# airframesio/aero-cli

Measured on AMD Instinct MI355X. Metric: Msamples/s demod+Viterbi, 10500bps OQPSK, 1/2/4/8 GPU; ACARS frames bit-exact vs ref, higher is better.
Workload: dtype f64

## Files before the change

### aero-cli_amd/build.py

```python
import argparse
import concurrent.futures as cf
import os
import shutil
import subprocess
import sys

HERE = os.path.dirname(os.path.abspath(__file__))
ROOT = os.path.dirname(HERE)
CSRC = os.path.join(HERE, 'csrc')
BUILD = os.path.join(HERE, 'build')
ENGINE_SO = os.path.join(HERE, 'libaero_engine.so')
SYNTH_SO = os.path.join(ROOT, 'tools', 'libaero_synth.so')
ORACLE_DIR = os.path.join(ROOT, 'oracle')

ARCH = os.environ.get('AERO_OFFLOAD_ARCH', 'gfx950')
HIPCC = os.environ.get('HIPCC', shutil.which('hipcc') or '/opt/rocm/bin/hipcc')
FP = ['-ffp-contract=off', '-fno-fast-math']
HIP_FLAGS = ['-O3', '-std=c++17', '-fPIC', '--offload-arch=' + ARCH] + FP
CXX_FLAGS = ['-O2', '-std=c++17', '-fPIC', '-Wall'] + FP

HIP_SRCS = ['demod_oqpsk.hip', 'demod_msk.hip', 'coarse.hip', 'aerol.hip', 'engine.hip', 'chan.hip', 'burst.hip', 'burst_msk.hip',
            'burst_engine.hip', 'cchan.hip', 'slot_reset.hip', 'slot_copy.hip']
CXX_SRCS = ['tables_host.cpp', 'acars_host.cpp', 'chan_blob.cpp']
FILE_FLAGS = {'burst.hip': ['-mllvm', '-disable-machine-licm'],
# ... 41 lines not shown
        for f in [ex.submit(_run, t) for t in tasks]:
            f.result()
    if tasks or _stale(out, objs):
        _run([HIPCC, '--offload-arch=' + ARCH, '-shared', '-fPIC', '-o', out] + objs)
    return out


def build_synth():
    src = os.path.join(ROOT, 'tools', 'aero_synth.cpp')
    if _stale(SYNTH_SO, [src]):
        _run(['g++', '-O2', '-std=c++17', '-fPIC', '-shared', '-o', SYNTH_SO, src, '-lm'])
    return SYNTH_SO


MATHHOST_SO = os.path.join(ROOT, 'tools', 'libaero_mathhost.so')
FFTSIM_SO = os.path.join(ROOT, 'tools', 'libfft_chain_sim.so')


def build_fftsim():
    src = os.path.join(ROOT, 'tools', 'fft_chain_sim.cpp')
    if _stale(FFTSIM_SO, [src, os.path.join(CSRC, 'fft_layout.h')]):
        _run(['g++', '-O2', '-std=c++17', '-fPIC', '-shared', '-ffp-contract=off', '-o', FFTSIM_SO, src])
    return FFTSIM_SO


SCHEDSIM_SO = os.path.join(ROOT, 'tools', 'libcoarse_sched_sim.so')


def build_schedsim():
    src = os.path.join(ROOT, 'tools', 'coarse_sched_sim.cpp')
    if _stale(SCHEDSIM_SO, [src, os.path.join(CSRC, 'coarse_sched.h')]):
        _run(['g++', '-O2', '-std=c++17', '-Wall', '-fPIC', '-shared', '-o', SCHEDSIM_SO, src])
    return SCHEDSIM_SO


CHANSLOTS_SO = os.path.join(ROOT, 'tools', 'libchan_slots_sim.so')


def build_chanslots():
    src = os.path.join(ROOT, 'tools', 'chan_slots_sim.cpp')
    if _stale(CHANSLOTS_SO, [src, os.path.join(CSRC, 'chan_slots.h')]):
        _run(['g++', '-O2', '-std=c++17', '-Wall', '-fPIC', '-shared', '-o', CHANSLOTS_SO, src])
    return CHANSLOTS_SO


def build_mathhost():
    src = os.path.join(ROOT, 'tools', 'mathhost.cpp')
    deps = [src, os.path.join(CSRC, 'aero_math.h'), os.path.join(CSRC, 'aero_glibc_tables.h')]
    if _stale(MATHHOST_SO, deps):
        _run(['g++', '-O2', '-std=c++17', '-fPIC', '-shared', '-ffp-contract=off', '-o', MATHHOST_SO, src, '-lm'])
    return MATHHOST_SO


HOSTCHECK_SO = os.path.join(ROOT, 'tools', 'libaero_hostcheck.so')
HOSTCHECK_SRCS = [os.path.join(ROOT, 'tools', 'hostcheck.cpp'), os.path.join(CSRC, 'acars_host.cpp'),
                  os.path.join(CSRC, 'chan_blob.cpp'), os.path.join(CSRC, 'tables_host.cpp')]


def build_hostcheck(out=HOSTCHECK_SO, extra=()):
    deps = HOSTCHECK_SRCS + [os.path.join(CSRC, h) for h in ('acars_host.h', 'chan_blob.h', 'tables_host.h')]
    if _stale(out, deps):
        _run(['g++'] + CXX_FLAGS + list(extra) + ['-shared', '-o', out] + HOSTCHECK_SRCS + ['-lm'])
    return out


def build_oracle():
# ... 59 lines not shown
    base = ['g++', '-O1', '-std=c++17', '-fPIC'] + FP + SAN
    out = {}
    jobsl = []
    def lib(name, srcs, extra=()):
        so = os.path.join(d, name)
        out[name] = so
        if _stale(so, srcs + [os.path.join(CSRC, 'aero_math.h'), os.path.join(CSRC, 'aero_glibc_tables.h')]):
            jobsl.append(base + list(extra) + ['-shared', '-o', so] + srcs + ['-lm'])
    lib('liboracle.so', [os.path.join(ORACLE_DIR, 'aero_oracle.cpp'), os.path.join(ORACLE_DIR, 'pub_oracle.cpp')])
    lib('libaero_synth.so', [os.path.join(ROOT, 'tools', 'aero_synth.cpp')])
    lib('libaero_mathhost.so', [os.path.join(ROOT, 'tools', 'mathhost.cpp')])
    lib('libaero_hostcheck.so', HOSTCHECK_SRCS)
    hs = [os.path.join(HOST, s) for s in HOST_COMMON]
    lib(os.path.join('bin', 'libaero_host.so'), [os.path.join(HOST, 'host_capi.cpp')] + hs[:2])
    for name, srcs in HOST_BINS.items():
        exe = os.path.join(bindir, name)
        out[name] = exe
        allsrc = [os.path.join(HOST, s) for s in srcs] + hs
        if _stale(exe, allsrc + [ENGINE_SO]):
            jobsl.append(base + ['-o', exe] + allsrc + [ENGINE_SO, '-Wl,-rpath,' + HERE, '-rdynamic', '-ldl',
                                                          '-lpthread'])
    with cf.ThreadPoolExecutor(max_workers=max(1, jobs)) as ex:
        for f in [ex.submit(_run, t) for t in jobsl]:
            f.result()
    return out


def build_all(jobs=4):
    build_oracle()
    build_synth()
    build_mathhost()
    build_fftsim()
    build_schedsim()
    build_chanslots()
    build_hostcheck()
    so = build_engine(jobs)
    build_diag(jobs)
    build_host(jobs)
    return so


DIAG_VARIANTS = {'handoff_fail': ['AERO_X_HANDOFF_FAIL']}


def build_diag(jobs=4):
    return [build_engine(jobs, variant=v, defines=d) for v, d in DIAG_VARIANTS.items()]


DROP_VARIANTS = {'drop%d' % k: ['AERO_X_DROP=%d' % k] for k in (1, 2, 4, 8)}


def build_drop(jobs=4):
    return [build_engine(jobs, variant=v, defines=d) for v, d in DROP_VARIANTS.items()]


BLIBM_VARIANTS = {'blibm%d' % k: ['AERO_X_BURST_LIBM=%d' % k] for k in (1, 2, 3)}


def build_blibm(jobs=4):
    return [build_engine(jobs, variant=v, defines=d) for v, d in BLIBM_VARIANTS.items()]


COARSE_VARIANTS = {'cisline': ['AERO_X_CISLINE'], 'noyread': ['AERO_X_NOYREAD']}


def build_coarse(jobs=4):
# ... 34 lines not shown
```

### aero-cli_amd/csrc/aero_math.h

```cpp
#pragma once
#include <stdint.h>

#if defined(__HIPCC__)
#include <hip/hip_runtime.h>
#define AERO_HD __host__ __device__ __forceinline__
#define AERO_TABLE_DECL static __host__ __device__ constexpr
#else
#include <math.h>
#define AERO_HD static inline
#define AERO_TABLE_DECL static constexpr
#endif

#include "aero_glibc_tables.h"

namespace aero {

AERO_HD uint64_t d2u(double x) { return __builtin_bit_cast(uint64_t, x); }
AERO_HD double u2d(uint64_t u) { return __builtin_bit_cast(double, u); }
AERO_HD uint32_t hiw(double x) { return (uint32_t)(d2u(x) >> 32); }
AERO_HD uint32_t low(double x) { return (uint32_t)d2u(x); }
AERO_HD double sethi(double x, uint32_t hi) {
  return u2d((d2u(x) & 0xffffffffULL) | ((uint64_t)hi << 32));
}
AERO_HD double mkd(uint32_t hi, uint32_t lo) { return u2d(((uint64_t)hi << 32) | lo); }
// ... 643 lines not shown
  const double du = div_r((a - vb) - vvb, b, r);
  const bool pos = x > 0;
  const bool prim = pos && gt;
  const bool cpi = !pos && !(ay > ax);
  const double K = cpi ? AERO_G_OPI : AERO_G_HPI, K1 = cpi ? AERO_G_OPI1 : AERO_G_HPI1;
  const double s = (!pos && ay > ax) ? 1.0 : -1.0;
  const double vs = u * u;
  const double poly = g_atan2_poly(vs);
  const double uv = u * vs;
  const double zp_s = u + fma(uv, poly, du);
  const double zz = uv * poly;
  const double ts = K + s * u;
  const double cor = (K - ts) + s * u;
  const double zg_s = (((cor + K1) + s * du) + s * zz) + ts;
  int row = g_atan2_row(u);
  row = row < 0 ? 0 : row;
  const double *c = cij[row];
  const double t3 = u - c[0];
  const double v = t3 + du;
  const double dv = (__builtin_fabs(t3) > __builtin_fabs(du)) ? ((t3 - v) + du) : ((du - v) + t3);
  double p3 = fma(v, c[6], c[5]);
  p3 = fma(v, p3, c[4]);
  p3 = fma(v, p3, c[3]);
  const double zp_t = fma(v, c[2], fma(dv, c[2], (v * v) * p3)) + c[1];
  const double P = fma(v, p3, c[2]);
  const double zg_t = (K + s * c[1]) + fma(s * v, P, K1);
  const double z = u < AERO_G_INV16 ? (prim ? zp_s : zg_s) : (prim ? zp_t : zg_t);
  return __builtin_copysign(z, y);
#else
  return aero_atan2_t(y, x, cij);
#endif
}

AERO_HD double aero_log(double x) {
  const uint64_t ix = d2u(x);
  const uint32_t top = (uint32_t)(ix >> 48);
  if (ix - 0x3fee000000000000ULL < 0x3090000000000ULL) {
    if (ix == 0x3ff0000000000000ULL) return 0.0;
    const double *B = aero_g_log_poly1;
    const double r = x - 1.0;
    const double r2 = r * r, r3 = r * r2;
    double p9 = fma(r3, B[10], fma(r2, B[9], fma(r, B[8], B[7])));
    p9 = fma(p9, r3, fma(r2, B[6], fma(r, B[5], B[4])));
    const double p = fma(p9, r3, fma(r2, B[3], fma(r, B[2], B[1])));
    const double rhi = fma(-AERO_G_TWO27, r, fma(r, AERO_G_TWO27, r));
    const double rlo = r - rhi;
    const double hi = fma(rhi * rhi, B[0], r);
    double lo = fma(rhi * rhi, B[0], r - hi);
    lo = fma(B[0] * rlo, r + rhi, lo);
    return hi + fma(p, r3, lo);
  }
  uint64_t jx = ix;
  if (top - 0x0010u >= 0x7ff0u - 0x0010u) {
    if ((ix << 1) == 0) return -1.0 / 0.0;
    if (ix == 0x7ff0000000000000ULL) return x;
    if ((top & 0x8000u) || (top & 0x7ff0u) == 0x7ff0u) return (x - x) / (x - x);
    jx = d2u(x * 0x1p52) - (52ULL << 52);
  }
  const uint64_t tmp = jx - 0x3fe6000000000000ULL;
  const int i = (int)((tmp >> 45) & 127);
  const int k = (int)((int64_t)tmp >> 52);
  const double z = u2d(jx - (tmp & (0xfffULL << 52)));
  const double invc = aero_g_log_tab[i][0], logc = aero_g_log_tab[i][1];
  const double r = fma(z, invc, -1.0);
  const double kd = (double)k;
  const double w = fma(kd, AERO_G_LN2HI, logc);
  const double hi = w + r;
  const double lo = fma(kd, AERO_G_LN2LO, (w - hi) + r);
  const double r2 = r * r;
  const double *A = aero_g_log_poly;
  const double q = fma(fma(r, A[4], A[3]), r2, fma(r, A[2], A[1]));
  return fma(r * r2, q, fma(r2, A[0], lo)) + hi;
}

AERO_HD double aero_log10(double x) {
  const double two54 = 0x1p54;
  int64_t ix = (int64_t)d2u(x);
  int64_t k;
  if (ix > 0x000fffffffffffffLL) {
    k = -1023;
  } else {
    if ((ix & 0x7fffffffffffffffLL) == 0) return -two54 / __builtin_fabs(x);
    if (ix < 0) return (x - x) / (x - x);
    x *= two54;
    ix = (int64_t)d2u(x);
    k = -1023 - 54;
  }
  if ((uint64_t)ix > 0x7fefffffffffffffULL) return x + x;
  k += ix >> 52;
  const int64_t i = (int64_t)((uint64_t)k >> 63);
  const double y = (double)(k + i);
  x = u2d((uint64_t)(ix & 0x000fffffffffffffLL) | ((uint64_t)(0x3ff - i) << 52));
  const double z = y * AERO_G_LOG10_2LO + aero_log(x) * AERO_G_IVLN10;
  return z + y * AERO_G_LOG10_2HI;
}

}
```

### aero-cli_amd/csrc/coarse.hip

```cpp
#include <hip/hip_runtime.h>

#include <type_traits>

#include "aero_math.h"
#include "coarse_sched.h"
#include "engine_common.h"
#include "fft_chain.h"

namespace aero {

#ifdef AERO_X_OCML
#define CO_HYPOT ::hypot
#define CO_HYPOT_NR ::hypot
#define CO_LOG10 ::log10
#else
#define CO_HYPOT aero_hypot
#define CO_HYPOT_NR aero_hypot_nr
#define CO_LOG10 aero_log10
#endif

template <int M>
struct CoarseK;
template <>
struct CoarseK<MODE_OQPSK> {
  static constexpr int LOG2N = 14, HOPN = 4096, START = 3584, STOP = 12800, ILO = 4608, IHI = 11776, EPB = 1792;
  static constexpr int YLO = 2815, YHI = 13568;
  static constexpr double FS = 48000.0;
};
template <>
struct CoarseK<MODE_C8400> {
  static constexpr int LOG2N = 14, HOPN = 4096, START = 3584, STOP = 12800, ILO = 4608, IHI = 11776, EPB = 1434;
  static constexpr int YLO = 2815, YHI = 13568;
  static constexpr double FS = 48000.0;
};
template <int FS>
struct MskCoarseBins;
template <>
struct MskCoarseBins<12000> {
  static constexpr int START = 614, STOP = 7578, ILO = 3482, IHI = 4710, EPB = 205;
};
template <>
struct MskCoarseBins<24000> {
  static constexpr int START = 307, STOP = 7885, ILO = 3789, IHI = 4403, EPB = 102;
};
template <>
struct MskCoarseBins<48000> {
  static constexpr int START = 154, STOP = 8038, ILO = 3942, IHI = 4250, EPB = 51;
};
template <int M>
struct CoarseK {
  using B = MskCoarseBins<msk_fs(M)>;
  static constexpr int LOG2N = 13, HOPN = 2048, START = B::START, STOP = B::STOP, ILO = B::ILO, IHI = B::IHI,
                       EPB = B::EPB;
  static constexpr int YLO = MSK_YLO, YHI = MSK_YHI;
  static_assert(ILO - EPB - 1 >= YLO && IHI - 1 + EPB + 1 <= YHI, "fold search inside the kept y bins");
  static constexpr double FS = (double)msk_fs(M);
};

struct CoarseBins {
  int start, stop, ilo, ihi, epb;
  double fs;
};
template <int M>
__device__ __forceinline__ CoarseBins coarse_bins(const DevState &S) {
  using K = CoarseK<M>;
// ... 147 lines not shown
__device__ __forceinline__ HopPro load_pro(const DevState &S, int C, int c) {
  HopPro p;
  p.filled = S.ls[LS_FILLED * C + c];
  p.zero_before = S.ls[LS_ZERO_BEFORE * C + c];
  p.hops_done = S.is[IS_HOPS_DONE * C + c];
  p.yreset = S.is[IS_YRESET * C + c];
  return p;
}
__device__ __forceinline__ HopPro uni(const HopPro &p) {
  return {uni(p.filled), uni(p.zero_before), uni(p.hops_done), uni(p.yreset)};
}

struct HopEpi {
  double mse, m2f, m2s, mcf, mcs;
  int ecd, countdown2, countdown, iter, scans, steps, hop_n;
};
__device__ __forceinline__ HopEpi load_epi(const DevState &S, int C, int c) {
  HopEpi e;
  e.mse = S.ds[DS_MSE * C + c];
  e.m2f = S.ds[DS_M2_FREQ * C + c];
  e.m2s = S.ds[DS_M2_STEP * C + c];
  e.mcf = S.ds[DS_MC_FREQ * C + c];
  e.mcs = S.ds[DS_MC_STEP * C + c];
  e.ecd = S.is[IS_EMPTYCD * C + c];
  e.countdown2 = S.is[IS_COUNTDOWN2 * C + c];
  e.countdown = S.is[IS_COUNTDOWN * C + c];
  e.iter = S.is[IS_HUNT_ITER * C + c];
  e.scans = S.is[IS_HUNT_SCANS * C + c];
  e.steps = S.is[IS_HUNT_STEPS * C + c];
  e.hop_n = S.hop_n[c];
  return e;
}

template <int M>
__global__ __launch_bounds__(1 << (CoarseK<M>::LOG2N - 4), CoarseK<M>::LOG2N == 13 ? 4 : 1) void coarse_kernel(DevState S, DevTables T, int nch) {
  using K = CoarseK<M>;
  const CoarseBins KB = coarse_bins<M>(S);
  constexpr int L = K::LOG2N, N = 1 << L, FT = N / 16, PADDED = N + N / 16;
  constexpr int YLEN = K::YHI - K::YLO + 1;
  constexpr bool PERSIST = L == 14;
  __shared__ double lds[PADDED];
  __shared__ double2 s_tw[TwLds<L>::LEN];
  __shared__ double red_v[FT / 64];
  __shared__ int red_i[FT / 64];
  const int wave = uni((int)threadIdx.x >> 6);
  const int C = S.C;
  const int wgs = (int)gridDim.x, wg = (int)blockIdx.x;
  const int iters = csched::iters(nch, wgs, wg);
#ifdef AERO_X_STAMPS
  unsigned long long cst_[CSTAMP_N] = {}, ctime_ = __builtin_amdgcn_s_memtime();
  const unsigned long long cstart_ = ctime_;
#endif
  bool have_tw = false;
#pragma unroll 1
  for (int k0 = 0; k0 < iters; k0 += csched::BATCH) {
    bool due = false;
    if (csched::lane_has(iters, k0, lane_now())) {
      const int cc = csched::channel(wgs, wg, k0 + lane_now());
      const long long nsamp = S.ls[LS_NSAMP * C + cc];
      const long long avail = S.ls[LS_AVAIL * C + cc];
      const long long nkk = (long long)K::HOPN * (S.is[IS_HOPS_DONE * C + cc] + 1) - 1;
      due = nsamp == nkk && avail > nkk;
    }
    unsigned long long mask = __ballot(due);
    HopPro pro{};
    bool have_pro = false;
#pragma unroll 1
    while (mask) {
      auto tnow = [&]() { return wave * 64 + lane_now(); };
      int t = PERSIST ? tnow() : (int)threadIdx.x;
      const int c = csched::channel(wgs, wg, k0 + csched::first(mask));
      mask = csched::rest(mask);
      if (!have_pro) pro = uni(load_pro(S, C, c));
      const long long filled = pro.filled, zero_before = pro.zero_before;
      const int hops_done = pro.hops_done, yreset = pro.yreset;
      const long long nk = (long long)K::HOPN * (hops_done + 1) - 1;
      int fixj = -1;
      uint32_t fixw = 0;
      if (filled <= nk) {
        const double mc_ptr = S.ds[DS_MC_PTR * C + c];
        int tint = (int)mc_ptr;
        if (tint >= WTSIZE) tint = 0;
        if (tint < 0) tint = WTSIZE - 1;
        const int16_t xs = S.pcm[(nk & (S.pcm_cap - 1)) * C + c];
        fixw = (uint32_t)tint | ((uint32_t)(uint16_t)xs << 16);
        fixj = (int)(nk & (N - 1));
        if (t == 0) {
          S.cring[(size_t)c * N + fixj] = fixw;
          S.ls[LS_FILLED * C + c] = nk + 1;
        }
      }
      CSTAMP(0);

      if (!have_tw) {
        load_tw_lds<L>(s_tw, T.tw, t, FT);
        have_tw = true;
      }
      uint32_t *ring_lds = reinterpret_cast<uint32_t *>(lds);
      const uint32_t *ring = S.cring + (size_t)c * N;
      if constexpr (PERSIST) {
#pragma unroll
        for (int i = 0; i < N / FT; ++i) {
          const int j = t + i * FT;
          const uint32_t w = ring[j];
          ring_lds[j + (j >> 4)] = j == fixj ? fixw : w;
        }
      } else {
        for (int j = t; j < N; j += FT) {
          const uint32_t w = ring[j];
          ring_lds[j + (j >> 4)] = j == fixj ? fixw : w;
        }
      }
      __syncthreads();
      CSTAMP(1);
      double2 x[16];
      const long long s0 = nk - (N - 1);
      double2 cs[16];
      double dval[16];
#pragma unroll
      for (int i = 0; i < 16; ++i) {
        const int q = (int)((s0 + bitrev<L>(epos<L, 0>(t, i))) & (N - 1));
        const uint32_t w = ring_lds[q + (q >> 4)];
        dval[i] = ((double)(int16_t)(w >> 16)) / 32768.0;
#ifdef AERO_X_CISLINE
        cs[i] = T.cis[w & 0x7];
#else
        cs[i] = T.cis[w & 0xFFFF];
#endif
      }
#pragma unroll
      for (int i = 0; i < 16; ++i) asm volatile("" : "+v"(cs[i].x), "+v"(cs[i].y));
#pragma unroll
      for (int i = 0; i < 16; ++i) {
        const long long s = s0 + bitrev<L>(epos<L, 0>(t, i));
        x[i] = s < zero_before ? make_double2(0.0, 0.0) : make_double2(cs[i].x * dval[i], cs[i].y * dval[i]);
      }
      __syncthreads();
      CSTAMP(2);
      if constexpr (PERSIST) t = tnow();
      chain::fft<L, true, false>(x, t, lds, T.tw, s_tw, T.twg);
      CSTAMP(3);
      if constexpr (PERSIST) t = tnow();
      const int bin_t = chain::out_bin_thread<L>(t);
#pragma unroll
      for (int i = 0; i < 16; ++i) {
        const int p = bin_t | chain::out_bin_reg<L>(i);
        if constexpr (M == MODE_C8400) {
          const double w = T.cwin[i * FT + t];
          x[i] = make_double2(x[i].x * w, x[i].y * w);
        } else {
          if (p >= KB.start && p <= KB.stop) x[i] = make_double2(0.0, 0.0);
        }
      }
      if constexpr (PERSIST) t = tnow();
      chain::fft<L, false, true>(x, t, lds, T.twi, s_tw, T.twgi);
#pragma unroll
      for (int i = 0; i < 16; ++i) {
        const double r = x[i].x * x[i].x - x[i].y * x[i].y;
        const double im = 2.0 * (x[i].x * x[i].y);
        x[i] = make_double2(r, im);
      }
      CSTAMP(4);
      if constexpr (PERSIST) t = tnow();
      chain::fft<L, false, false>(x, t, lds, T.tw, s_tw, T.twg);
      CSTAMP(5);
      if constexpr (PERSIST) t = tnow();
      double *yg = S.y + (size_t)c * YLEN;
#ifdef AERO_X_NOYREAD
      auto yload = [&](int k) { return 20.0 + 0.0 * k; };
#else
      auto yload = [&](int k) { return (k < YLEN && !yreset) ? yg[k] : 20.0; };
#endif
      double yp0 = yload(t), yp1 = yload(t + FT);
      double *ylds = lds;
      auto ypad = [](int q) { return fftl::ypadn<6>(q); };
      bool nr = true;
#pragma unroll
      for (int i = 0; i < 16; ++i) {
        const double a = fabs(x[i].x), b = fabs(x[i].y);
        nr = nr && a <= 0x1p200 && b <= 0x1p200 && (a >= 0x1p-200 || b >= 0x1p-200);
      }
      if (__all(nr)) {
#pragma unroll
        for (int i = 0; i < 16; ++i) {
          const int yi = (bin_t | chain::out_bin_reg<L>(i)) ^ (N / 2);
          if (yi >= K::YLO && yi <= K::YHI) ylds[ypad(yi - K::YLO)] = CO_HYPOT_NR(x[i].x, x[i].y);
        }
      } else {
#pragma unroll
        for (int i = 0; i < 16; ++i) {
          const int yi = (bin_t | chain::out_bin_reg<L>(i)) ^ (N / 2);
          if (yi >= K::YLO && yi <= K::YHI) ylds[ypad(yi - K::YLO)] = CO_HYPOT(x[i].x, x[i].y);
        }
      }
      double yp2 = yload(t + 2 * FT);
      __syncthreads();
      CSTAMP(6);
      have_pro = mask != 0;
      HopPro pn{};
      if (have_pro) pn = load_pro(S, C, csched::channel(wgs, wg, k0 + csched::first(mask)));
      HopEpi ep{};
      if (PERSIST && t < 64) ep = load_epi(S, C, c);
#pragma unroll 1
      for (int k = t; k < YLEN; k += FT) {
        const double yold = yp0;
        yp0 = yp1;
        yp1 = yp2;
        yp2 = yload(k + 3 * FT);
        const double ynew = yold * 0.9 + 0.1 * 10 * CO_LOG10(fmax(ylds[ypad(k)], 1.0));
        yg[k] = ynew;
        ylds[ypad(k)] = ynew;
      }
      __syncthreads();
      CSTAMP(7);
      double bv = 0.0;
      int bi = 0x7fffffff;
      for (int r = 0;; ++r) {
        const int i = KB.ilo + t + FT * r;
        if (i >= KB.ihi) break;
        double val = 0;
        for (int j = -1; j <= 1; j++)
          val += (ylds[ypad(i - KB.epb - j - K::YLO)] + ylds[ypad(i + KB.epb + j - K::YLO)]);
        if (val > bv) {
          bv = val;
          bi = i;
        }
      }
      for (int off = 32; off > 0; off >>= 1) {
        const double ov = __shfl_down(bv, off, 64);
        const int oi = __shfl_down(bi, off, 64);
        if (ov > bv || (ov == bv && oi < bi)) {
          bv = ov;
          bi = oi;
        }
      }
      if ((t & 63) == 0) {
        red_v[t >> 6] = bv;
        red_i[t >> 6] = bi;
      }
      if (have_pro) pro = uni(pn);
      __syncthreads();
      CSTAMP(8);
      if (t == 0) {
        if constexpr (!PERSIST) ep = load_epi(S, C, c);
        for (int w = 1; w < FT / 64; ++w) {
          if (red_v[w] > bv || (red_v[w] == bv && red_i[w] < bi)) {
            bv = red_v[w];
            bi = red_i[w];
          }
        }
        const int zmaxloc = (bv > 0.0) ? bi : N / 2;
        const double nfft = (double)N;
        const double freq_offset_est = -((double)(zmaxloc - nfft / 2)) * (KB.fs / nfft) * 0.5;
        double est;
        int ecd = ep.ecd;
        if (ecd <= 0) {
          est = freq_offset_est;
        } else {
          ecd--;
          est = 0;
        }

        double *ds = S.ds;
        int *is = S.is;
        const double mse = ep.mse;
        HopCtl h;
        h.m2f = ep.m2f;
        h.m2s = ep.m2s;
        h.mcf = ep.mcf;
        h.mcs = ep.mcs;
        h.countdown2 = ep.countdown2;
        h.countdown = ep.countdown;
        h.ecd = ecd;
        h.yres_next = 0;
        h.zb = zero_before;
// ... 27 lines not shown
          hr[2] = h.m2f;
          hr[3] = h.mcf;
          hr[4] = mse;
          hr[5] = gotasignal ? 1.0 : 0.0;
        }
        S.hop_n[c] = hn + 1;
      }
      CSTAMP(9);
#ifdef AERO_X_STAMPS
      cst_[CSTAMP_N - 1]++;
#endif
      if constexpr (!PERSIST) break;
    }
    if constexpr (!PERSIST) break;
  }
#ifdef AERO_X_STAMPS
  if (wave * 64 + lane_now() == 0 && cst_[CSTAMP_N - 1]) {
    cst_[10] = __builtin_amdgcn_s_memtime() - cstart_;
    for (int k = 0; k < CSTAMP_N; ++k) atomicAdd(&g_cstamps[k], cst_[k]);
  }
#endif
}

void coarse_read_stamps(unsigned long long *out) {
#ifdef AERO_X_STAMPS
  (void)hipMemcpyFromSymbol(out, HIP_SYMBOL(g_cstamps), sizeof(unsigned long long) * CSTAMP_N);
  unsigned long long z[CSTAMP_N] = {0};
  (void)hipMemcpyToSymbol(HIP_SYMBOL(g_cstamps), z, sizeof z);
#else
  for (int k = 0; k < CSTAMP_N; ++k) out[k] = 0;
#endif
}

void launch_coarse(hipStream_t st, int mode, const DevState &S, const DevTables &T, int nch, int grid) {
  const dim3 pg(csched::grid(nch, grid < 1 ? 1 : grid));
  switch (mode) {
    case MODE_OQPSK: hipLaunchKernelGGL(coarse_kernel<MODE_OQPSK>, pg, dim3(1024), 0, st, S, T, nch); break;
    case MODE_C8400: hipLaunchKernelGGL(coarse_kernel<MODE_C8400>, pg, dim3(1024), 0, st, S, T, nch); break;
    case MODE_MSK600: hipLaunchKernelGGL(coarse_kernel<MODE_MSK600>, dim3(nch), dim3(512), 0, st, S, T, nch); break;
    case MODE_MSK1200: hipLaunchKernelGGL(coarse_kernel<MODE_MSK1200>, dim3(nch), dim3(512), 0, st, S, T, nch); break;
    case MODE_MSK600_24K:
      hipLaunchKernelGGL(coarse_kernel<MODE_MSK600_24K>, dim3(nch), dim3(512), 0, st, S, T, nch);
      break;
    case MODE_MSK600_48K:
      hipLaunchKernelGGL(coarse_kernel<MODE_MSK600_48K>, dim3(nch), dim3(512), 0, st, S, T, nch);
      break;
    case MODE_MSK1200_12K:
      hipLaunchKernelGGL(coarse_kernel<MODE_MSK1200_12K>, dim3(nch), dim3(512), 0, st, S, T, nch);
      break;
    case MODE_MSK1200_48K:
      hipLaunchKernelGGL(coarse_kernel<MODE_MSK1200_48K>, dim3(nch), dim3(512), 0, st, S, T, nch);
      break;
    default:
      hipLaunchKernelGGL(coarse_kernel<MODE_MSKG600>, dim3(nch), dim3(512), 0, st, S, T, nch);
      break;
  }
}

}
```

### aero-cli_amd/csrc/engine.hip

```cpp
#include <hip/hip_runtime.h>

#include <algorithm>
#include <cmath>
#include <complex>
#include <cstdio>
#include <cstdlib>
#include <cstring>
#include <atomic>
#include <chrono>
#include <climits>
#include <deque>
#include <condition_variable>
#include <functional>
#include <mutex>
#include <new>
#include <map>
#include <memory>
#include <string>
#include <set>
#include <thread>
#include <type_traits>
#include <vector>

#include "../../include/aero_engine.h"
#include "acars_host.h"
#include "burst_engine.h"
#include "aero_math.h"
#include "chan_blob.h"
#include "engine_common.h"
#include "fft_layout.h"
#include "host_pool.h"
#include "engine_internal.h"
#include "slot_copy.h"
#include "slot_reset.h"
#include "tables_host.h"

namespace aero {
void launch_demod(hipStream_t, const DevState &, const DevTables &, int, int, bool, bool);
void upload_demod_constants(const double *, const DelayDesc *, const double *, const double *, const double *,
                            const double *);
void launch_demod_msk(hipStream_t, int, const DevState &, const DevTables &, int, int, bool);
void upload_msk_constants(const double *);
void demod_read_stamps(unsigned long long *);
void coarse_read_stamps(unsigned long long *);
void viterbi_read_stamps(unsigned long long *);
void burst_read_stamps(unsigned long long *);
void launch_coarse(hipStream_t, int, const DevState &, const DevTables &, int, int);
void launch_frame(hipStream_t, int, const DevState &, int);
void launch_viterbi(hipStream_t, int, const DevState &, const DevTables &, int, int);
void launch_prefilter_c(hipStream_t, const DevState &, const DevTables &, const void *, int);
void launch_demod_c(hipStream_t, const DevState &, const DevTables &, int, bool);
void upload_c_constants(const DelayDesc *);
int c_prejob_bytes();
void launch_reset_slots(hipStream_t, void *, const ResetSeg *, int, const int *, const int *, int, const ResetInit *,
                        unsigned long long);
}

using namespace aero;

namespace {

constexpr int GENERIC_GROUP_CAP = 256;
constexpr long long PCM_CAP = 65536;
constexpr int PT_CAP = 4096;
constexpr int HOP_CAP = 64;

#define HIPCHK(x)                                   \
  do {                                              \
    hipError_t err__ = (x);                         \
    if (err__ != hipSuccess) {                      \
      fprintf(stderr, "aero_engine: %s failed: %s\n", #x, hipGetErrorString(err__)); \
      return AERO_E_HIP;                            \
    }                                               \
  } while (0)

__global__ void pcm_scatter_kernel(int16_t *ring, int C, long long capm, const int16_t *src, long long n, long long ld,
                                   int nch, int c0, long long start) {
  const long long total = n * nch;
  for (long long k = blockIdx.x * (long long)blockDim.x + threadIdx.x; k < total;
       k += (long long)gridDim.x * blockDim.x) {
// ... 49 lines not shown

struct TimingSlot {
  double ms = 0;
  long launches = 0;
};

struct HostTimer {
  std::map<std::string, TimingSlot> *t;
  const char *name;
  std::chrono::steady_clock::time_point t0;
  HostTimer(std::map<std::string, TimingSlot> *tm, const char *n) : t(tm), name(n) {
    if (t) t0 = std::chrono::steady_clock::now();
  }
  ~HostTimer() {
    if (!t) return;
    auto &slot = (*t)[name];
    slot.ms += std::chrono::duration<double, std::milli>(std::chrono::steady_clock::now() - t0).count();
    slot.launches++;
  }
};
#define HT_CAT2(a, b) a##b
#define HT_CAT(a, b) HT_CAT2(a, b)
#define HOST_TIMER(e, n) HostTimer HT_CAT(_ht_, __LINE__)(((e)->flags & AERO_F_TIMING) ? &(e)->timing : nullptr, n)

}


struct Group {
  ~Group();
  int mode = MODE_OQPSK;
  int gid = 0;
  int wide_max = 0;
  int coarse_grid = 1;
  ModeGeom g{};
  int device = 0, flags = 0, C = 0, nch = 0;
  std::string tag;
  hipStream_t st = nullptr;
  DevState S{};
  DevTables T{};
  void *pool = nullptr;
  size_t pool_bytes = 0;
  HostPool *hpool = nullptr;
  std::vector<aero_channel_cfg> cfg;
  std::vector<int> gch;
  std::vector<int> free_slots;
  std::vector<int> reset_pending;
  std::vector<uint8_t> reset_wait;
  std::vector<ResetSeg> reset_plan;
  ResetSeg *d_reset_plan = nullptr;
  ResetInit *d_reset_init = nullptr;
  int *d_reset_slots = nullptr, *pin_reset_slots = nullptr;
  hipEvent_t reset_ev = nullptr;
  bool reset_done = false, reset_ready = false;
  uint64_t reset_launches = 0;
  SlotCopier copier;
  std::vector<ResetSeg> slot_plan;
  std::vector<long long> avail, nsamp, hops;
  std::vector<std::unique_ptr<PChannelHost>> host;
  std::vector<std::vector<uint8_t>> infofield;
  std::vector<std::vector<int16_t>> soft_hold;
  std::vector<std::vector<double>> hop_hold, pt_hold;
  std::vector<std::vector<uint8_t>> blk_hold, frame_hold;
  std::vector<long long> soft_seen;
  std::vector<long long> hop_base;
  int job_out = JOB_OUT;
  std::vector<std::deque<long long>> msg_end;
// ... 678 lines not shown
          waited = true;
        }
        jt[ncj++] = {c, 0, e->pre_end[c], e->msg_end[c].front()};
        e->pre_end[c] = e->msg_end[c].front();
        e->msg_end[c].pop_front();
      }
      if (ncj) e->next_cjob = (kcj + 1) % Group::NPIN;
    }
    for (int c = 0; c < e->nch; c++) {
      const long long boundary = HOPN * (e->hops[c] + 1) - 1;
      if (e->nsamp[c] == boundary && e->avail[c] > boundary) {
        e->hops[c]++;
        any_hop = true;
      }
    }
    for (int c = 0; c < e->nch; c++) {
      const long long boundary = HOPN * (e->hops[c] + 1) - 1;
      long long end = std::min(e->avail[c], boundary);
      if (!flush && e->avail[c] <= boundary) end = e->nsamp[c];
      if (cch) end = std::min(e->pre_end[c], boundary);
      if (end > e->nsamp[c]) {
        e->processed += (uint64_t)(end - e->nsamp[c]);
        e->nsamp[c] = end;
        progress = true;
      }
    }
    if (!any_hop && !progress && !ncj) {
      *more = false;
      return AERO_OK;
    }
    hipEvent_t a, b;
    if (any_hop) {
      ev_begin(e, "coarse", a, b);
      launch_coarse(e->st, e->mode, e->S, e->T, e->nch, e->coarse_grid);
      ev_end(e, b);
    }
    if (int rc = issue_viterbi(e)) return rc;
    if (ncj) {
      HIPCHK(hipMemcpyAsync(e->d_cjobs[kcj], e->pin_cjobs[kcj], (size_t)c_prejob_bytes() * ncj,
                            hipMemcpyHostToDevice, e->st));
      HIPCHK(hipEventRecord(e->cjob_ev[kcj], e->st));
      ev_begin(e, "prefilter", a, b);
      launch_prefilter_c(e->st, e->S, e->T, e->d_cjobs[kcj], ncj);
      ev_end(e, b);
      HIPCHK(hipGetLastError());
    }
    if (!progress) return AERO_OK;
    ev_begin(e, "demod", a, b);
    if (cch)
      launch_demod_c(e->st, e->S, e->T, e->nch, (e->flags & AERO_F_TRACE_PT) != 0);
    else if (e->mode == MODE_OQPSK)
      launch_demod(e->st, e->S, e->T, e->nch, flush, (e->flags & AERO_F_TRACE_PT) != 0, e->nch <= e->wide_max);
    else
      launch_demod_msk(e->st, e->mode, e->S, e->T, e->nch, flush, e->nch <= e->wide_max);
    ev_end(e, b);
    if (int rc = note_consumed(e)) return rc;
    if (int rc = frame_round(e, flush, trace)) return rc;
    if (flush && e->S.dcd_tick)
      if (int rc = frame_round(e, flush, trace)) return rc;
  }
  return AERO_OK;
}

int frame_round(Group *e, int flush, bool trace) {
  hipEvent_t a, b;
  {
    const int si = e->next_slot;
// ... 121 lines not shown
  const double nfft = MSK_NFFT, hzperbin = (double)fs / nfft, lockingbw = 900.0, fb = 600.0;
  const double startbin = std::max(std::round(lockingbw / hzperbin), 1.0);
  m.start = (int)startbin;
  m.stop = (int)(nfft - startbin);
  m.epb = (int)std::round(fb / (2.0 * hzperbin));
  m.ilo = (int)std::round((-lockingbw / hzperbin) + ((double)(MSK_NFFT / 2)));
  m.ihi = (int)std::round((lockingbw / hzperbin) + ((double)(MSK_NFFT / 2)));
  return m.ilo - m.epb - 1 >= MSK_YLO && m.ihi - 1 + m.epb + 1 <= MSK_YHI && m.ilo < m.ihi;
}

constexpr int WIDE_MAX_DEFAULT = 4096;

int group_create(aero_engine *E, int mode, int gid, int fs, std::unique_ptr<Group> &out) {
  std::unique_ptr<Group> e(new Group());
  e->mode = mode;
  e->gid = gid;
  e->device = E->device;
  e->flags = E->flags;
  e->hpool = E->hpool.get();
  MskGen mg{};
  if (mode != MODE_OQPSK && mode != MODE_C8400) {
    if (!msk_gen_consts(msk_generic(mode) ? fs : msk_fs(mode), mg)) return AERO_E_RATE;
  }
  {
    const char *w = getenv(mode == MODE_OQPSK ? "AERO_OQPSK_WIDE" : "AERO_MSK_WIDE");
    e->wide_max = w ? atoi(w) : WIDE_MAX_DEFAULT;
    const char *cg = getenv("AERO_COARSE_GRID");
    int cus = 0;
    if (cg)
      cus = atoi(cg);
    else
      HIPCHK(hipDeviceGetAttribute(&cus, hipDeviceAttributeMultiprocessorCount, e->device));
    e->coarse_grid = std::max(cus, 1);
  }
  if (msk_generic(mode)) {
    e->g = msk_geom(msk_bitrate(mode), fs);
    e->tag = "msk" + std::to_string(msk_bitrate(mode)) + "_" + std::to_string(fs) + "_";
  } else if (mode == MODE_C8400) {
    e->g = mode_geom(mode);
    e->tag = "c8400_";
    e->job_out = JOB_OUT_C;
  } else {
    static const char *const tags[MODE_COUNT] = {"", "msk600_", "msk1200_", "msk600_24k_", "msk600_48k_",
                                                  "msk1200_12k_", "msk1200_48k_"};
    e->g = mode_geom(mode);
    e->tag = tags[mode];
  }
  e->C = (E->capacity(msk_generic(mode) ? mode : gid, msk_generic(mode) ? fs : 0) + 63) & ~63;
  if (msk_generic(mode)) e->C = std::min(e->C, GENERIC_GROUP_CAP);
  DevState S{};
  DevTables T{};
  const size_t bytes = layout(S, T, mode, e->g, e->C, e->flags, nullptr) + 4096;
  if (hipMalloc(&e->pool, bytes) != hipSuccess) return AERO_E_NOMEM;
  e->pool_bytes = bytes;
  HIPCHK(hipMemset(e->pool, 0, bytes));
  layout(e->S, e->T, mode, e->g, e->C, e->flags, reinterpret_cast<char *>(e->pool));
  e->S.mg = mg;
  HIPCHK(hipStreamCreateWithFlags(&e->st, hipStreamNonBlocking));
  if (hipHostMalloc(&e->h_err, 64, hipHostMallocMapped | hipHostMallocCoherent) != hipSuccess) return AERO_E_NOMEM;
  *e->h_err = 0;
  HIPCHK(hipHostGetDevicePointer((void **)&e->h_err_dev, e->h_err, 0));
  e->S.err = e->h_err_dev;
  for (auto &sl : e->slot) {
    if (hipMalloc(&sl.d_n, 64) != hipSuccess) return AERO_E_NOMEM;
    if (hipHostMalloc(&sl.h_out, (size_t)e->job_out * e->C, hipHostMallocMapped | hipHostMallocCoherent) != hipSuccess)
      return AERO_E_NOMEM;
// ... 1566 lines not shown
```

Measured before the change: 9013.

## Overlap next channel's ring load and gather with coarse spectrum tail

```diff
diff --git a/aero-cli_amd/build.py b/aero-cli_amd/build.py
--- a/aero-cli_amd/build.py
+++ b/aero-cli_amd/build.py
@@ -97,6 +97,16 @@
     if _stale(SCHEDSIM_SO, [src, os.path.join(CSRC, 'coarse_sched.h')]):
         _run(['g++', '-O2', '-std=c++17', '-Wall', '-fPIC', '-shared', '-o', SCHEDSIM_SO, src])
     return SCHEDSIM_SO
+
+
+LDSSIM_SO = os.path.join(ROOT, 'tools', 'libcoarse_lds_sim.so')
+
+
+def build_ldssim():
+    src = os.path.join(ROOT, 'tools', 'coarse_lds_sim.cpp')
+    if _stale(LDSSIM_SO, [src, os.path.join(CSRC, 'coarse_lds.h')]):
+        _run(['g++', '-O2', '-std=c++17', '-Wall', '-fPIC', '-shared', '-o', LDSSIM_SO, src])
+    return LDSSIM_SO
 
 
 CHANSLOTS_SO = os.path.join(ROOT, 'tools', 'libchan_slots_sim.so')
@@ -222,6 +232,7 @@
     build_mathhost()
     build_fftsim()
     build_schedsim()
+    build_ldssim()
     build_chanslots()
     build_hostcheck()
     so = build_engine(jobs)
diff --git a/aero-cli_amd/csrc/aero_math.h b/aero-cli_amd/csrc/aero_math.h
--- a/aero-cli_amd/csrc/aero_math.h
+++ b/aero-cli_amd/csrc/aero_math.h
@@ -699,7 +699,7 @@
 #endif
 }
 
-AERO_HD double aero_log(double x) {
+AERO_HD double aero_log_tab(double x, const double *tab) {
   const uint64_t ix = d2u(x);
   const uint32_t top = (uint32_t)(ix >> 48);
   if (ix - 0x3fee000000000000ULL < 0x3090000000000ULL) {
@@ -728,7 +728,7 @@
   const int i = (int)((tmp >> 45) & 127);
   const int k = (int)((int64_t)tmp >> 52);
   const double z = u2d(jx - (tmp & (0xfffULL << 52)));
-  const double invc = aero_g_log_tab[i][0], logc = aero_g_log_tab[i][1];
+  const double invc = tab[2 * i], logc = tab[2 * i + 1];
   const double r = fma(z, invc, -1.0);
   const double kd = (double)k;
   const double w = fma(kd, AERO_G_LN2HI, logc);
@@ -740,7 +740,9 @@
   return fma(r * r2, q, fma(r2, A[0], lo)) + hi;
 }
 
-AERO_HD double aero_log10(double x) {
+AERO_HD double aero_log(double x) { return aero_log_tab(x, &aero_g_log_tab[0][0]); }
+
+AERO_HD double aero_log10_tab(double x, const double *tab) {
   const double two54 = 0x1p54;
   int64_t ix = (int64_t)d2u(x);
   int64_t k;
@@ -758,8 +760,9 @@
   const int64_t i = (int64_t)((uint64_t)k >> 63);
   const double y = (double)(k + i);
   x = u2d((uint64_t)(ix & 0x000fffffffffffffLL) | ((uint64_t)(0x3ff - i) << 52));
-  const double z = y * AERO_G_LOG10_2LO + aero_log(x) * AERO_G_IVLN10;
+  const double z = y * AERO_G_LOG10_2LO + aero_log_tab(x, tab) * AERO_G_IVLN10;
   return z + y * AERO_G_LOG10_2HI;
 }
-
-}
+AERO_HD double aero_log10(double x) { return aero_log10_tab(x, &aero_g_log_tab[0][0]); }
+
+}
diff --git a/aero-cli_amd/csrc/coarse.hip b/aero-cli_amd/csrc/coarse.hip
--- a/aero-cli_amd/csrc/coarse.hip
+++ b/aero-cli_amd/csrc/coarse.hip
@@ -3,6 +3,7 @@
 #include <type_traits>
 
 #include "aero_math.h"
+#include "coarse_lds.h"
 #include "coarse_sched.h"
 #include "engine_common.h"
 #include "fft_chain.h"
@@ -13,10 +14,12 @@
 #define CO_HYPOT ::hypot
 #define CO_HYPOT_NR ::hypot
 #define CO_LOG10 ::log10
+#define CO_LOG10_TAB(x, tab) ::log10(x)
 #else
 #define CO_HYPOT aero_hypot
 #define CO_HYPOT_NR aero_hypot_nr
 #define CO_LOG10 aero_log10
+#define CO_LOG10_TAB(x, tab) aero_log10_tab(x, tab)
 #endif
 
 template <int M>
@@ -24,13 +27,13 @@
 template <>
 struct CoarseK<MODE_OQPSK> {
   static constexpr int LOG2N = 14, HOPN = 4096, START = 3584, STOP = 12800, ILO = 4608, IHI = 11776, EPB = 1792;
-  static constexpr int YLO = 2815, YHI = 13568;
+  static constexpr int YLO = clds::YLO14, YHI = clds::YHI14;
   static constexpr double FS = 48000.0;
 };
 template <>
 struct CoarseK<MODE_C8400> {
   static constexpr int LOG2N = 14, HOPN = 4096, START = 3584, STOP = 12800, ILO = 4608, IHI = 11776, EPB = 1434;
-  static constexpr int YLO = 2815, YHI = 13568;
+  static constexpr int YLO = clds::YLO14, YHI = clds::YHI14;
   static constexpr double FS = 48000.0;
 };
 template <int FS>
@@ -244,17 +247,47 @@
   return e;
 }
 
-template <int M>
+template <int L, int YLEN, bool OVL>
+struct CoarseLds {
+  double *lds;
+  double2 *s_tw;
+  double *red_v;
+  int *red_i;
+  uint32_t *img;
+  double *logtab;
+};
+template <int L, int YLEN, bool OVL>
+__device__ __forceinline__ CoarseLds<L, YLEN, OVL> coarse_lds() {
+  using LM = clds::Map<L, YLEN, OVL>;
+  static_assert(LM::TWLEN == TwLds<L>::LEN && clds::ypad(12345) == fftl::ypadn<6>(12345), "coarse_lds.h restates these");
+  if constexpr (OVL) {
+    __shared__ __attribute__((aligned(16))) unsigned char raw[LM::TOTAL];
+    return {reinterpret_cast<double *>(raw + LM::LDS_OFF), reinterpret_cast<double2 *>(raw + LM::TW_OFF),
+            reinterpret_cast<double *>(raw + LM::REDV_OFF), reinterpret_cast<int *>(raw + LM::REDI_OFF),
+            reinterpret_cast<uint32_t *>(raw + LM::IMG_OFF), reinterpret_cast<double *>(raw + LM::LOGTAB_OFF)};
+  } else {
+    __shared__ double lds[LM::PADDED];
+    __shared__ double2 s_tw[LM::TWLEN];
+    __shared__ double red_v[LM::FT / 64];
+    __shared__ int red_i[LM::FT / 64];
+    static_assert(sizeof lds + sizeof s_tw + sizeof red_v + sizeof red_i == LM::TOTAL, "coarse_lds.h describes this");
+    return {lds, s_tw, red_v, red_i, nullptr, nullptr};
+  }
+}
+
+template <int M, bool OVL = false>
 __global__ __launch_bounds__(1 << (CoarseK<M>::LOG2N - 4), CoarseK<M>::LOG2N == 13 ? 4 : 1) void coarse_kernel(DevState S, DevTables T, int nch) {
   using K = CoarseK<M>;
   const CoarseBins KB = coarse_bins<M>(S);
-  constexpr int L = K::LOG2N, N = 1 << L, FT = N / 16, PADDED = N + N / 16;
+  constexpr int L = K::LOG2N, N = 1 << L, FT = N / 16;
   constexpr int YLEN = K::YHI - K::YLO + 1;
   constexpr bool PERSIST = L == 14;
-  __shared__ double lds[PADDED];
-  __shared__ double2 s_tw[TwLds<L>::LEN];
-  __shared__ double red_v[FT / 64];
-  __shared__ int red_i[FT / 64];
+  static_assert(PERSIST || !OVL, "the overlapped head belongs to the persistent walk");
+  const auto sm = coarse_lds<L, YLEN, OVL>();
+  double *const lds = sm.lds;
+  double2 *const s_tw = sm.s_tw;
+  double *const red_v = sm.red_v;
+  int *const red_i = sm.red_i;
   const int wave = uni((int)threadIdx.x >> 6);
   const int C = S.C;
   const int wgs = (int)gridDim.x, wg = (int)blockIdx.x;
@@ -277,6 +310,8 @@
     unsigned long long mask = __ballot(due);
     HopPro pro{};
     bool have_pro = false;
+    bool pre = false;
+    double2 x[16];
 #pragma unroll 1
     while (mask) {
       auto tnow = [&]() { return wave * 64 + lane_now(); };
@@ -287,68 +322,78 @@
       const long long filled = pro.filled, zero_before = pro.zero_before;
       const int hops_done = pro.hops_done, yreset = pro.yreset;
       const long long nk = (long long)K::HOPN * (hops_done + 1) - 1;
-      int fixj = -1;
-      uint32_t fixw = 0;
-      if (filled <= nk) {
-        const double mc_ptr = S.ds[DS_MC_PTR * C + c];
-        int tint = (int)mc_ptr;
-        if (tint >= WTSIZE) tint = 0;
-        if (tint < 0) tint = WTSIZE - 1;
-        const int16_t xs = S.pcm[(nk & (S.pcm_cap - 1)) * C + c];
-        fixw = (uint32_t)tint | ((uint32_t)(uint16_t)xs << 16);
-        fixj = (int)(nk & (N - 1));
-        if (t == 0) {
-          S.cring[(size_t)c * N + fixj] = fixw;
-          S.ls[LS_FILLED * C + c] = nk + 1;
-        }
-      }
-      CSTAMP(0);
-
-      if (!have_tw) {
-        load_tw_lds<L>(s_tw, T.tw, t, FT);
-        have_tw = true;
-      }
-      uint32_t *ring_lds = reinterpret_cast<uint32_t *>(lds);
-      const uint32_t *ring = S.cring + (size_t)c * N;
-      if constexpr (PERSIST) {
-#pragma unroll
-        for (int i = 0; i < N / FT; ++i) {
-          const int j = t + i * FT;
-          const uint32_t w = ring[j];
-          ring_lds[j + (j >> 4)] = j == fixj ? fixw : w;
-        }
-      } else {
-        for (int j = t; j < N; j += FT) {
-          const uint32_t w = ring[j];
-          ring_lds[j + (j >> 4)] = j == fixj ? fixw : w;
-        }
-      }
-      __syncthreads();
-      CSTAMP(1);
-      double2 x[16];
+      auto ring_fixup = [&](int cc, long long fil, long long nkk, int tt, int &fj, uint32_t &fw) {
+        fj = -1;
+        fw = 0;
+        if (fil <= nkk) {
+          const double mc_ptr = S.ds[DS_MC_PTR * C + cc];
+          int tint = (int)mc_ptr;
+          if (tint >= WTSIZE) tint = 0;
+          if (tint < 0) tint = WTSIZE - 1;
+          const int16_t xs = S.pcm[(nkk & (S.pcm_cap - 1)) * C + cc];
+          fw = (uint32_t)tint | ((uint32_t)(uint16_t)xs << 16);
+          fj = (int)(nkk & (N - 1));
+          if (tt == 0) {
+            S.cring[(size_t)cc * N + fj] = fw;
+            S.ls[LS_FILLED * C + cc] = nkk + 1;
+          }
+        }
+      };
       const long long s0 = nk - (N - 1);
-      double2 cs[16];
-      double dval[16];
-#pragma unroll
-      for (int i = 0; i < 16; ++i) {
-        const int q = (int)((s0 + bitrev<L>(epos<L, 0>(t, i))) & (N - 1));
-        const uint32_t w = ring_lds[q + (q >> 4)];
-        dval[i] = ((double)(int16_t)(w >> 16)) / 32768.0;
+      if (!(OVL && pre)) {
+        int fixj;
+        uint32_t fixw;
+        ring_fixup(c, filled, nk, t, fixj, fixw);
+        CSTAMP(0);
+
+        if (!have_tw) {
+          load_tw_lds<L>(s_tw, T.tw, t, FT);
+          if constexpr (OVL)
+            if (t < 256) sm.logtab[t] = (&aero_g_log_tab[0][0])[t];
+          have_tw = true;
+        }
+        uint32_t *ring_lds = reinterpret_cast<uint32_t *>(lds);
+        const uint32_t *ring = S.cring + (size_t)c * N;
+        if constexpr (PERSIST) {
+#pragma unroll
+          for (int i = 0; i < N / FT; ++i) {
+            const int j = t + i * FT;
+            const uint32_t w = ring[j];
+            ring_lds[j + (j >> 4)] = j == fixj ? fixw : w;
+          }
+        } else {
+          for (int j = t; j < N; j += FT) {
+            const uint32_t w = ring[j];
+            ring_lds[j + (j >> 4)] = j == fixj ? fixw : w;
+          }
+        }
+        __syncthreads();
+        CSTAMP(1);
+        double2 cs[16];
+        double dval[16];
+#pragma unroll
+        for (int i = 0; i < 16; ++i) {
+          const int q = (int)((s0 + bitrev<L>(epos<L, 0>(t, i))) & (N - 1));
+          const uint32_t w = ring_lds[q + (q >> 4)];
+          dval[i] = ((double)(int16_t)(w >> 16)) / 32768.0;
 #ifdef AERO_X_CISLINE
-        cs[i] = T.cis[w & 0x7];
+          cs[i] = T.cis[w & 0x7];
 #else
-        cs[i] = T.cis[w & 0xFFFF];
-#endif
-      }
-#pragma unroll
-      for (int i = 0; i < 16; ++i) asm volatile("" : "+v"(cs[i].x), "+v"(cs[i].y));
-#pragma unroll
-      for (int i = 0; i < 16; ++i) {
-        const long long s = s0 + bitrev<L>(epos<L, 0>(t, i));
-        x[i] = s < zero_before ? make_double2(0.0, 0.0) : make_double2(cs[i].x * dval[i], cs[i].y * dval[i]);
-      }
-      __syncthreads();
-      CSTAMP(2);
+          cs[i] = T.cis[w & 0xFFFF];
+#endif
+        }
+#pragma unroll
+        for (int i = 0; i < 16; ++i) asm volatile("" : "+v"(cs[i].x), "+v"(cs[i].y));
+#pragma unroll
+        for (int i = 0; i < 16; ++i) {
+          const long long s = s0 + bitrev<L>(epos<L, 0>(t, i));
+          x[i] = s < zero_before ? make_double2(0.0, 0.0) : make_double2(cs[i].x * dval[i], cs[i].y * dval[i]);
+        }
+        __syncthreads();
+        CSTAMP(2);
+      }
+      const bool nxt = mask != 0;
+      const int cn = nxt ? csched::channel(wgs, wg, k0 + csched::first(mask)) : c;
       if constexpr (PERSIST) t = tnow();
       chain::fft<L, true, false>(x, t, lds, T.tw, s_tw, T.twg);
       CSTAMP(3);
@@ -366,17 +411,41 @@
       }
       if constexpr (PERSIST) t = tnow();
       chain::fft<L, false, true>(x, t, lds, T.twi, s_tw, T.twgi);
+      HopPro pn{};
+      if constexpr (OVL) pn = load_pro(S, C, cn);
 #pragma unroll
       for (int i = 0; i < 16; ++i) {
         const double r = x[i].x * x[i].x - x[i].y * x[i].y;
         const double im = 2.0 * (x[i].x * x[i].y);
         x[i] = make_double2(r, im);
       }
+      if constexpr (OVL) pn = uni(pn);
       CSTAMP(4);
       if constexpr (PERSIST) t = tnow();
       chain::fft<L, false, false>(x, t, lds, T.tw, s_tw, T.twg);
       CSTAMP(5);
       if constexpr (PERSIST) t = tnow();
+      uint32_t rw[16];
+      uint32_t pcmw[8];
+      int fixjn = -1;
+      uint32_t fixwn = 0;
+      const long long nkn = (long long)K::HOPN * (pn.hops_done + 1) - 1;
+      if (OVL && nxt) ring_fixup(cn, pn.filled, nkn, t, fixjn, fixwn);
+      if constexpr (OVL) {
+        __builtin_amdgcn_s_waitcnt(0x0F70);
+      }
+      auto ring_issue = [&]() {
+        if constexpr (OVL) {
+          if (nxt) {
+            const uint32_t *ringn = S.cring + (size_t)cn * N + fresh(t);
+#pragma unroll
+            for (int i = 0; i < N / FT; ++i) rw[i] = ringn[i * FT];
+          } else {
+#pragma unroll
+            for (int i = 0; i < N / FT; ++i) rw[i] = 0;
+          }
+        }
+      };
       double *yg = S.y + (size_t)c * YLEN;
 #ifdef AERO_X_NOYREAD
       auto yload = [&](int k) { return 20.0 + 0.0 * k; };
@@ -395,36 +464,129 @@
       if (__all(nr)) {
 #pragma unroll
         for (int i = 0; i < 16; ++i) {
+          if (i == 8) ring_issue();
           const int yi = (bin_t | chain::out_bin_reg<L>(i)) ^ (N / 2);
           if (yi >= K::YLO && yi <= K::YHI) ylds[ypad(yi - K::YLO)] = CO_HYPOT_NR(x[i].x, x[i].y);
         }
       } else {
 #pragma unroll
         for (int i = 0; i < 16; ++i) {
+          if (i == 8) ring_issue();
           const int yi = (bin_t | chain::out_bin_reg<L>(i)) ^ (N / 2);
           if (yi >= K::YLO && yi <= K::YHI) ylds[ypad(yi - K::YLO)] = CO_HYPOT(x[i].x, x[i].y);
+        }
+      }
+      if constexpr (OVL) {
+        if (nxt) {
+          using LM = clds::Map<L, YLEN, OVL>;
+#pragma unroll
+          for (int i = 0; i < N / FT; ++i) {
+            const int j = t + i * FT;
+            sm.img[LM::img(j)] = j == fixjn ? fixwn : rw[i];
+          }
         }
       }
       double yp2 = yload(t + 2 * FT);
       __syncthreads();
       CSTAMP(6);
-      have_pro = mask != 0;
-      HopPro pn{};
-      if (have_pro) pn = load_pro(S, C, csched::channel(wgs, wg, k0 + csched::first(mask)));
+      have_pro = nxt;
+      if constexpr (!OVL)
+        if (have_pro) pn = load_pro(S, C, cn);
       HopEpi ep{};
-      if (PERSIST && t < 64) ep = load_epi(S, C, c);
-#pragma unroll 1
-      for (int k = t; k < YLEN; k += FT) {
+      if (PERSIST && !OVL && t < 64) ep = load_epi(S, C, c);
+      double2 twv;
+      auto ycalc = [&](double yold, int k) {
+        double lg;
+        if constexpr (OVL)
+          lg = CO_LOG10_TAB(fmax(ylds[ypad(k)], 1.0), sm.logtab);
+        else
+          lg = CO_LOG10(fmax(ylds[ypad(k)], 1.0));
+        const double ynew = yold * 0.9 + 0.1 * 10 * lg;
+        if constexpr (!OVL) yg[k] = ynew;
+        ylds[ypad(k)] = ynew;
+      };
+      auto ybody = [&](int k) {
         const double yold = yp0;
         yp0 = yp1;
         yp1 = yp2;
         yp2 = yload(k + 3 * FT);
-        const double ynew = yold * 0.9 + 0.1 * 10 * CO_LOG10(fmax(ylds[ypad(k)], 1.0));
-        yg[k] = ynew;
-        ylds[ypad(k)] = ynew;
+        ycalc(yold, k);
+      };
+      const long long s0n = nkn - (N - 1);
+      auto gather4 = [&](auto i0c) {
+        if constexpr (OVL) {
+          using LM = clds::Map<L, YLEN, OVL>;
+          constexpr int i0 = decltype(i0c)::value;
+          if (nxt) {
+#pragma unroll
+            for (int i = i0; i < i0 + 4; ++i) {
+              const int q = (int)((s0n + bitrev<L>(epos<L, 0>(t, i))) & (N - 1));
+              const uint32_t w = sm.img[LM::img(q)];
+              pcmw[i >> 1] = (i & 1) ? (pcmw[i >> 1] | (w & 0xFFFF0000u)) : (w >> 16);
+#ifdef AERO_X_CISLINE
+              x[i] = T.cis[w & 0x7];
+#else
+              x[i] = T.cis[w & 0xFFFF];
+#endif
+            }
+          } else {
+#pragma unroll
+            for (int i = i0; i < i0 + 4; ++i) {
+              x[i] = T.cis[0];
+              pcmw[i >> 1] = 0;
+            }
+          }
+        }
+      };
+      if constexpr (OVL) {
+        static_assert((YLEN + FT - 1) / FT <= 12, "four groups of three iterations cover the bins");
+        twv = make_double2(0.0, 0.0);
+        constexpr int NIT = (YLEN + FT - 1) / FT;
+        auto ystep = [&](double &yp, auto jc) {
+          constexpr int j = decltype(jc)::value;
+          constexpr bool full = (j + 1) * FT <= YLEN;
+          static_assert(full || j >= NIT - 1, "one partial iteration, the last");
+          if constexpr (j < NIT) {
+            const int k = t + j * FT;
+            if (full || uni(k) < YLEN) {
+              const bool in = full || k < YLEN;
+#ifdef AERO_X_NOYREAD
+              double a = 20.0 * 0.9;
+#else
+              double a = ((in && !yreset) ? yp : 20.0) * 0.9;
+              asm volatile("" : "+v"(a));
+              if constexpr (j + 3 < NIT) yp = yg[min(k + 3 * FT, YLEN - 1)];
+#endif
+              const double lg = CO_LOG10_TAB(fmax(ylds[ypad(in ? k : YLEN - 1)], 1.0), sm.logtab);
+              const double ynew = a + 0.1 * 10 * lg;
+              if (in) ylds[ypad(k)] = ynew;
+            }
+          }
+        };
+        auto ygroup = [&](auto i0c) {
+          constexpr int g = decltype(i0c)::value / 4;
+          if (g == 3) twv = T.tw[min(t, TwLds<L>::LEN - 1)];
+          gather4(i0c);
+          ystep(yp0, std::integral_constant<int, 3 * g>());
+          ystep(yp1, std::integral_constant<int, 3 * g + 1>());
+          ystep(yp2, std::integral_constant<int, 3 * g + 2>());
+        };
+        ygroup(std::integral_constant<int, 0>());
+        ygroup(std::integral_constant<int, 4>());
+        ygroup(std::integral_constant<int, 8>());
+        ygroup(std::integral_constant<int, 12>());
+      } else {
+#pragma unroll 1
+        for (int k = t; k < YLEN; k += FT) ybody(k);
       }
       __syncthreads();
       CSTAMP(7);
+      if constexpr (OVL) {
+        if (nxt && t < TwLds<L>::LEN) s_tw[t] = twv;
+#pragma unroll 1
+        for (int k = t; k < YLEN; k += FT) yg[k] = ylds[ypad(k)];
+        if (t < 64) ep = load_epi(S, C, c);
+      }
       double bv = 0.0;
       int bi = 0x7fffffff;
       for (int r = 0;; ++r) {
@@ -453,6 +615,21 @@
       if (have_pro) pro = uni(pn);
       __syncthreads();
       CSTAMP(8);
+      pre = OVL && nxt;
+      if constexpr (OVL) {
+        if (nxt) {
+#pragma unroll
+          for (int i = 0; i < 16; ++i) asm volatile("" : "+v"(x[i].x), "+v"(x[i].y));
+#pragma unroll
+          for (int i = 0; i < 16; ++i) {
+            const uint32_t pw = pcmw[i >> 1];
+            const double dv = ((double)(int16_t)((i & 1) ? (pw >> 16) : (pw & 0xFFFFu))) / 32768.0;
+            const long long s = s0n + bitrev<L>(epos<L, 0>(t, i));
+            x[i] = s < pn.zero_before ? make_double2(0.0, 0.0) : make_double2(x[i].x * dv, x[i].y * dv);
+          }
+        }
+        CSTAMP(2);
+      }
       if (t == 0) {
         if constexpr (!PERSIST) ep = load_epi(S, C, c);
         for (int w = 1; w < FT / 64; ++w) {
@@ -546,11 +723,21 @@
 #endif
 }
 
-void launch_coarse(hipStream_t st, int mode, const DevState &S, const DevTables &T, int nch, int grid) {
+void launch_coarse(hipStream_t st, int mode, const DevState &S, const DevTables &T, int nch, int grid, bool overlap) {
   const dim3 pg(csched::grid(nch, grid < 1 ? 1 : grid));
   switch (mode) {
-    case MODE_OQPSK: hipLaunchKernelGGL(coarse_kernel<MODE_OQPSK>, pg, dim3(1024), 0, st, S, T, nch); break;
-    case MODE_C8400: hipLaunchKernelGGL(coarse_kernel<MODE_C8400>, pg, dim3(1024), 0, st, S, T, nch); break;
+    case MODE_OQPSK:
+      if (overlap)
+        hipLaunchKernelGGL((coarse_kernel<MODE_OQPSK, true>), pg, dim3(1024), 0, st, S, T, nch);
+      else
+        hipLaunchKernelGGL((coarse_kernel<MODE_OQPSK, false>), pg, dim3(1024), 0, st, S, T, nch);
+      break;
+    case MODE_C8400:
+      if (overlap)
+        hipLaunchKernelGGL((coarse_kernel<MODE_C8400, true>), pg, dim3(1024), 0, st, S, T, nch);
+      else
+        hipLaunchKernelGGL((coarse_kernel<MODE_C8400, false>), pg, dim3(1024), 0, st, S, T, nch);
+      break;
     case MODE_MSK600: hipLaunchKernelGGL(coarse_kernel<MODE_MSK600>, dim3(nch), dim3(512), 0, st, S, T, nch); break;
     case MODE_MSK1200: hipLaunchKernelGGL(coarse_kernel<MODE_MSK1200>, dim3(nch), dim3(512), 0, st, S, T, nch); break;
     case MODE_MSK600_24K:
diff --git a/aero-cli_amd/csrc/coarse_lds.h b/aero-cli_amd/csrc/coarse_lds.h
--- /dev/null
+++ b/aero-cli_amd/csrc/coarse_lds.h
@@ -0,0 +1,40 @@
+#pragma once
+
+namespace aero {
+namespace clds {
+
+constexpr int ypad(int q) { return q + (q >> 6); }
+constexpr int tw_len(int log2n) { return 2 * (log2n >= 14 ? 512 : 256) - 1; }
+constexpr int YLO14 = 2815, YHI14 = 13568;
+
+constexpr int LDS_LIMIT = 160 * 1024;
+
+template <int L, int YLEN, bool OVL>
+struct Map {
+  static constexpr int N = 1 << L, FT = N / 16, PADDED = N + N / 16, TWLEN = tw_len(L);
+  static constexpr int YSPAN = ypad(YLEN - 1) + 1;
+  static constexpr int Y_BYTES = YSPAN * 8;
+  static constexpr int img(int j) { return j + (j >> 4); }
+  static constexpr int IMG_WORDS = img(N - 1) + 1;
+  static constexpr int IMG_OFF = Y_BYTES, IMG_BYTES = IMG_WORDS * 4, IMG_END = IMG_OFF + IMG_BYTES;
+
+  static constexpr int LDS_OFF = 0, LDS_BYTES = PADDED * 8;
+  static constexpr int TW_OFF = LDS_OFF + LDS_BYTES, TW_BYTES = TWLEN * 16;
+  static constexpr int SPARE_OFF = TW_OFF + TW_BYTES;
+  static constexpr int SPARE_BYTES = !OVL || IMG_END <= SPARE_OFF ? 0 : (IMG_END - SPARE_OFF + 7) / 8 * 8;
+  static constexpr int REDV_OFF = SPARE_OFF + SPARE_BYTES, REDV_BYTES = FT / 64 * 8;
+  static constexpr int REDI_OFF = REDV_OFF + REDV_BYTES, REDI_BYTES = FT / 64 * 4;
+  static constexpr int LOGTAB_OFF = (REDI_OFF + REDI_BYTES + 15) / 16 * 16, LOGTAB_BYTES = OVL ? 128 * 16 : 0;
+  static constexpr int TOTAL = OVL ? LOGTAB_OFF + LOGTAB_BYTES : REDI_OFF + REDI_BYTES;
+
+  static_assert(YSPAN <= PADDED, "ylds inside lds");
+  static_assert(TW_OFF % 16 == 0 && REDV_OFF % 8 == 0 && IMG_OFF % 4 == 0, "alignment");
+  static_assert(TOTAL <= LDS_LIMIT, "one workgroup's LDS");
+  static_assert(!OVL || IMG_OFF >= Y_BYTES, "image and ylds disjoint");
+  static_assert(!OVL || IMG_END <= REDV_OFF, "image and red_* disjoint");
+  static_assert(!OVL || IMG_END <= TW_OFF || IMG_END >= SPARE_OFF, "s_tw covered whole or not at all");
+  static_assert(!OVL || TWLEN <= FT, "one s_tw entry per thread");
+};
+
+}
+}
diff --git a/aero-cli_amd/csrc/engine.hip b/aero-cli_amd/csrc/engine.hip
--- a/aero-cli_amd/csrc/engine.hip
+++ b/aero-cli_amd/csrc/engine.hip
@@ -45,7 +45,7 @@
 void coarse_read_stamps(unsigned long long *);
 void viterbi_read_stamps(unsigned long long *);
 void burst_read_stamps(unsigned long long *);
-void launch_coarse(hipStream_t, int, const DevState &, const DevTables &, int, int);
+void launch_coarse(hipStream_t, int, const DevState &, const DevTables &, int, int, bool);
 void launch_frame(hipStream_t, int, const DevState &, int);
 void launch_viterbi(hipStream_t, int, const DevState &, const DevTables &, int, int);
 void launch_prefilter_c(hipStream_t, const DevState &, const DevTables &, const void *, int);
@@ -161,6 +161,7 @@
   int gid = 0;
   int wide_max = 0;
   int coarse_grid = 1;
+  bool coarse_overlap = true;
   ModeGeom g{};
   int device = 0, flags = 0, C = 0, nch = 0;
   std::string tag;
@@ -905,7 +906,7 @@
     hipEvent_t a, b;
     if (any_hop) {
       ev_begin(e, "coarse", a, b);
-      launch_coarse(e->st, e->mode, e->S, e->T, e->nch, e->coarse_grid);
+      launch_coarse(e->st, e->mode, e->S, e->T, e->nch, e->coarse_grid, e->coarse_overlap);
       ev_end(e, b);
     }
     if (int rc = issue_viterbi(e)) return rc;
@@ -1093,6 +1094,8 @@
     else
       HIPCHK(hipDeviceGetAttribute(&cus, hipDeviceAttributeMultiprocessorCount, e->device));
     e->coarse_grid = std::max(cus, 1);
+    const char *co = getenv("AERO_COARSE_OVERLAP");
+    e->coarse_overlap = !co || atoi(co) != 0;
   }
   if (msk_generic(mode)) {
     e->g = msk_geom(msk_bitrate(mode), fs);
```

New measurement: 9121, median of 6. 1.2% higher.
